# Huguet57/LIMO-Velo

Measured on NVIDIA B200. Metric: matched-points/sec per IESKF iteration (64k-pt sweep, 1M-pt map), higher is better.
Workload: dtype f32 geometry / f64 Jacobian+filter

## Files before the change

limo-velo_b200/csrc/lv_capi.cu:

```cuda
#include <math.h>
#include <stddef.h>
#include <stdio.h>
#include <stdlib.h>
#include <string.h>

#include <string>
#include <vector>

#include "../../include/limovelo_b200.h"
#include "lv_host.h"
#include "lv_internal.h"
#include "lv_predict.h"

using namespace lv;

static_assert(sizeof(lv_iter_log) == sizeof(IterLog), "lv_iter_log must mirror lv::IterLog");
static_assert(LV_MAX_EVALS == kMaxEvals, "log capacity");
static_assert(LV_STATE_LEN == kStateLen && LV_DOF == kDof, "state layout");

static thread_local std::string g_last_error;
static void set_error(const std::string& s) { g_last_error = s; }

#define LV_CUDA(call)                                                                            \
    do {                                                                                         \
// ... 122 lines not shown
}

static void fill_iprm(lv_context* h) {
    h->iprm.R = h->prm.LiDAR_noise;
    h->iprm.D = h->prm.degeneracy_threshold;
    for (int i = 0; i < kN; ++i) h->iprm.limits[i] = h->prm.LIMITS[i];
    h->iprm.max_iter = h->prm.MAX_NUM_ITERS;
    h->iprm.estimate_extrinsics = h->prm.estimate_extrinsics;
}

static MeasureArgs make_measure_args(lv_context* h, const float* d_xyz, int64_t n) {
    MeasureArgs a;
    memset(&a, 0, sizeof(a));
    a.xyz = d_xyz;
    a.n = (int32_t)n;
    a.n_tiles = (int32_t)((n + kMeasureThreads - 1) / kMeasureThreads);
    a.map = map_view(h->map);
    a.ctrl = h->d_ctrl;
    const double md = h->prm.MAX_DIST_PLANE;
    a.gate_d2 = md * md;
    float f = (float)a.gate_d2;
    if ((double)f < a.gate_d2) f = nextafterf(f, INFINITY);
    a.max_d2 = f;
    a.planes_threshold = h->prm.PLANES_THRESHOLD;
    a.estimate_extrinsics = h->prm.estimate_extrinsics;
    a.partials = h->d_partials;
    a.group_rows = h->d_group_rows;
    a.group_tickets = h->d_group_tickets;
    a.nn_a = h->d_nn_a;
    a.nn_b = h->d_nn_b;
    a.hard_list = h->d_hard_list;
    a.hard_seg = hard_segment(h->prm.max_points);
    a.hard_count = h->d_hard_list + (size_t)kHardBuckets * a.hard_seg;
    if (h->prm.sort_queries) {
        a.bin_key = h->d_bin_key; a.bin_val = h->d_bin_val; a.bin_key_in = h->d_bin_key_in; a.bin_val_in = h->d_bin_val_in;
        a.redo_flag = h->d_redo_flag;
        a.sort_tmp = h->d_bin_tmp; a.sort_tmp_bytes = h->bin_tmp_bytes;
        a.sort_bits = 0;
        for (uint32_t sl = h->map.slots; sl > 1; sl >>= 1) a.sort_bits++;
    }
    return a;
}

template <class T>
static cudaError_t ensure(T** p, size_t count) {
    if (*p) return cudaSuccess;
    return cudaMalloc(p, sizeof(T) * count);
}

extern "C" {

const char* lv_last_error(void) { return g_last_error.c_str(); }
const char* lv_version(void) { return "limovelo_b200 0.1 (sm_100a)"; }
int64_t lv_result_bytes(void) { return (int64_t)sizeof(UpdateCtrl); }

#define LV_CREATE_CUDA(call)                                                                     \
    do {                                                                                         \
        cudaError_t e__ = (call);                                                                \
        if (e__ != cudaSuccess) {                                                                \
            char buf__[512];                                                                     \
            snprintf(buf__, sizeof(buf__), "%s:%d: %s -> %s", __FILE__, __LINE__, #call,         \
                     cudaGetErrorString(e__));                                                   \
            lv_destroy(h);                                                                       \
            set_error(buf__);                                                                    \
            return LV_ERR_CUDA;                                                                  \
        }                                                                                        \
    } while (0)

lv_status lv_create(const lv_params* p, lv_handle* out) {
    if (!p || !out) return LV_ERR_ARG;
    *out = nullptr;
    if (p->NUM_MATCH_POINTS != 5) { set_error("NUM_MATCH_POINTS must be 5 (5x3 plane fit)"); return LV_ERR_ARG; }
    if (p->MAX_NUM_ITERS < 0 || p->MAX_NUM_ITERS + 1 > LV_MAX_EVALS) {
        set_error("MAX_NUM_ITERS out of range");
        return LV_ERR_ARG;
    }
    if (!(p->voxel_size > 0.f) || !(p->map_downsample_size > 0.f) || p->max_map_points <= 0 || p->max_points <= 0) {
        set_error("bad capacity / voxel_size / map_downsample_size");
        return LV_ERR_ARG;
    }
    if (p->max_map_points > (1ll << 24) || p->max_points > (1ll << 24)) { set_error("capacity beyond 2^24 points"); return LV_ERR_ARG; }
    if (!(p->MAX_DIST_PLANE > 0.0) || p->MAX_DIST_PLANE > 48.0 * (double)p->map_downsample_size) {
        set_error("MAX_DIST_PLANE must be positive and at most 48 map_downsample_size (ring search bound)");
        return LV_ERR_ARG;
    }
    int ndev = 0;
    if (cudaGetDeviceCount(&ndev) != cudaSuccess || ndev <= 0) {
        set_error("no CUDA device available (there is no CPU fallback)");
        return LV_ERR_CUDA;
    }
    LV_CUDA(cudaSetDevice(p->device));
    lv_context* h = new lv_context();
    h->prm = *p;
    memset(&h->prof, 0, sizeof(h->prof));
    memset(h->logs, 0, sizeof(h->logs));
    memset(&h->map, 0, sizeof(h->map));
    fill_iprm(h);
    if (p->stream) { h->stream = (cudaStream_t)p->stream; h->own_stream = false; }
    else { LV_CREATE_CUDA(cudaStreamCreateWithFlags(&h->stream, cudaStreamNonBlocking)); h->own_stream = true; }
    LV_CREATE_CUDA(map_alloc(h->map, p->max_map_points, p->max_points, p->voxel_size, p->map_downsample_size));
    { int l = 0; LV_CREATE_CUDA(map_clear(h->map, h->stream, &l)); }
    LV_CREATE_CUDA(cudaMalloc(&h->d_sweep, sizeof(float) * 3 * p->max_points));
    LV_CREATE_CUDA(cudaMalloc(&h->d_nn_a, sizeof(int4) * p->max_points));
    LV_CREATE_CUDA(cudaMalloc(&h->d_nn_b, sizeof(int2) * p->max_points));
    LV_CREATE_CUDA(cudaMalloc(&h->d_hard_list, sizeof(uint32_t) * ((size_t)kHardBuckets * hard_segment(p->max_points) + kCounters)));
    LV_CREATE_CUDA(cudaMalloc(&h->d_ref, sizeof(float4) * p->max_points));
    LV_CREATE_CUDA(cudaMalloc(&h->d_redo, sizeof(uint32_t) * (p->max_points + 64)));
// ... 323 lines not shown
        lv_context::UpdateGraph u;
        lv_status s = build_update_graph(h, cap, &u);
        if (s != LV_OK) return s;
        h->graphs.push_back(u);
        g = &h->graphs.back();
    }
    UpdateCtrl* c = h->d_ctrl;
    MeasureJob* job = h->d_job;
    int n32 = (int)n;
    uint32_t* counters = h->d_hard_list + (size_t)kHardBuckets * hard_segment(h->prm.max_points);
    void* args[5] = {&c, &job, &d_xyz, &n32, &counters};
    cudaKernelNodeParams kp = {};
    kp.func = const_cast<void*>(ieskf_begin_kernel_ptr());
    kp.gridDim = dim3(1, 1, 1);
    kp.blockDim = dim3(256, 1, 1);
    kp.kernelParams = args;
    LV_CUDA(cudaGraphExecKernelNodeSetParams(g->exec, g->begin_node, &kp));
    LV_CUDA(cudaGraphLaunch(g->exec, h->stream));
    h->prof.total_launches += 1 + 4 * (h->prm.MAX_NUM_ITERS + 1) + (h->use_reuse ? h->prm.MAX_NUM_ITERS : 0) + (h->prm.sort_queries ? 5 : 0);
    return LV_OK;
}

static lv_status enqueue_update_kernels(lv_context* h, const float* d_xyz, int64_t n, bool as_job) {
    const int pdl = (h->use_pdl && !h->profile) ? 1 : 0;
    uint32_t* counters = h->d_hard_list + (size_t)kHardBuckets * hard_segment(h->prm.max_points);
    LV_CUDA(launch_ieskf_begin(h->d_ctrl, as_job ? h->d_job : nullptr, d_xyz, (int)n, counters, h->stream));
    if (!as_job) h->prof.total_launches += 1;
    MeasureArgs a = update_measure_args(h, d_xyz, n, as_job);
    const int grid = measure_grid((int)n);
    if (a.bin_key) {
        int l = 0;
        LV_CUDA(launch_bin(a, h->stream, pdl, &l));
        if (!as_job) h->prof.total_launches += l;
    }
    for (int e = 0; e <= h->prm.MAX_NUM_ITERS; ++e) {
        EventPair ep;
        bool pr;
        LV_CUDA(launch_measure_timed(h, a, grid, as_job ? 0 : 1, e , (int)(h->update_seq % kNevalsRing), e, pdl));
        pr = prof_begin(h, 1, &ep);
        ep.upd = (int)(h->update_seq % kNevalsRing); ep.slot = e;
        LV_CUDA(launch_ieskf_step(h->d_ctrl, h->iprm, h->d_group_rows, partial_groups(grid), h->stream, pdl));
        if (pr) prof_end(h, &ep);
        if (!as_job) h->prof.total_launches += 4 + ((e > 0 && h->use_reuse) ? 1 : 0);
    }
    if (h->profile) {
        LV_CUDA(cudaMemcpyAsync(&h->h_nevals[h->update_seq % kNevalsRing], &h->d_ctrl->n_evals, sizeof(int32_t),
                                cudaMemcpyDeviceToHost, h->stream));
        h->update_seq++;
    }
    return LV_OK;
}

static lv_status fetch_results(lv_context* h) {
    LV_CUDA(cudaMemcpyAsync(h->h_ctrl, h->d_ctrl, sizeof(UpdateCtrl), cudaMemcpyDeviceToHost, h->stream));
    LV_CUDA(map_fetch_counters(h->map, h->stream));
    LV_CUDA(cudaStreamSynchronize(h->stream));
    const UpdateCtrl* c = h->h_ctrl;
    memcpy(h->x, c->x, sizeof(h->x));
    if (c->status == LV_OK) memcpy(h->P, c->P, sizeof(h->P));
    h->n_evals = c->n_evals;
    memcpy(h->logs, c->logs, sizeof(h->logs));
    h->last_status = c->status;
    h->state_dirty = false;
    h->pending_fetch = false;
    if (c->status == LV_OK && map_status_from_mirror(h) != LV_OK) return LV_ERR_CAPACITY;
    return (lv_status)c->status;
}

lv_status lv_correct(lv_handle h, const float* xyz, int64_t n, double time, lv_iter_log* logs, int32_t* n_evals,
                     double* x_out, double* P_out) {
    if (!h || !xyz || n <= 0) return LV_ERR_ARG;
    if (n_evals) *n_evals = 0;
    if (h->map.empty) return LV_EMPTY_MAP;
    if (n > h->prm.max_points) { set_error("sweep capacity exceeded"); return LV_ERR_CAPACITY; }
    LV_CUDA(cudaSetDevice(h->prm.device));
    LV_CUDA(cudaMemcpyAsync(h->d_sweep, xyz, sizeof(float) * 3 * n, cudaMemcpyHostToDevice, h->stream));
    lv_status s = enqueue_update(h, h->d_sweep, n);
    if (s != LV_OK) return s;
    h->last_sweep = h->d_sweep; h->last_sweep_n = n;
    s = fetch_results(h);
    h->last_time_updated = time;
    if (logs) memcpy(logs, h->logs, sizeof(lv_iter_log) * (size_t)h->n_evals);
    if (n_evals) *n_evals = h->n_evals;
    if (x_out) memcpy(x_out, h->x, sizeof(h->x));
    if (P_out) memcpy(P_out, h->P, sizeof(h->P));
    return s;
}

lv_status lv_correct_device(lv_handle h, const float* d_xyz, int64_t n, double time) {
    if (!h || !d_xyz || n <= 0) return LV_ERR_ARG;
    if (h->map.empty) return LV_EMPTY_MAP;
    LV_CUDA(cudaSetDevice(h->prm.device));
    lv_status s = enqueue_update(h, d_xyz, n);
    h->last_sweep = d_xyz; h->last_sweep_n = n;
    h->last_time_updated = time;
    h->pending_fetch = true;
    return s;
}

lv_status lv_last_logs(lv_handle h, lv_iter_log* logs, int32_t* n_evals) {
    if (!h) return LV_ERR_ARG;
    LV_CUDA(cudaSetDevice(h->prm.device));
    lv_status s = fetch_results(h);
    if (logs) memcpy(logs, h->logs, sizeof(lv_iter_log) * (size_t)h->n_evals);
    if (n_evals) *n_evals = h->n_evals;
    return s;
}
// ... 278 lines not shown
```

limo-velo_b200/csrc/lv_hd.h:

```cpp
#ifndef LV_HD_H_
#define LV_HD_H_

#include <math.h>
#include <stdint.h>

#if defined(__CUDACC__)
#define LV_HD __host__ __device__ __forceinline__
#define LV_HD_NOINLINE __host__ __device__ inline
#else
#define LV_HD inline
#define LV_HD_NOINLINE inline
#endif

namespace lv {

LV_HD float fmul(float a, float b) {
#if defined(__CUDA_ARCH__)
    return __fmul_rn(a, b);
#else
    return a * b;
#endif
}
LV_HD float fadd(float a, float b) {
#if defined(__CUDA_ARCH__)
    return __fadd_rn(a, b);
#else
    return a + b;
#endif
}
LV_HD float fsub(float a, float b) {
#if defined(__CUDA_ARCH__)
    return __fsub_rn(a, b);
#else
    return a - b;
#endif
}
LV_HD float fdiv(float a, float b) {
#if defined(__CUDA_ARCH__)
    return __fdiv_rn(a, b);
#else
    return a / b;
#endif
}
LV_HD float fsqrt(float a) {
#if defined(__CUDA_ARCH__)
    return __fsqrt_rn(a);
#else
    return sqrtf(a);
#endif
}
LV_HD double dmul(double a, double b) {
#if defined(__CUDA_ARCH__)
    return __dmul_rn(a, b);
#else
    return a * b;
#endif
}
LV_HD double dadd(double a, double b) {
#if defined(__CUDA_ARCH__)
    return __dadd_rn(a, b);
#else
    return a + b;
#endif
}
// ... 18 lines not shown
```

limo-velo_b200/csrc/lv_ieskf.h:

```cpp
#ifndef LV_IESKF_H_
#define LV_IESKF_H_

#include "lv_point_math.h"

namespace lv {

#ifndef LV_TK
#define LV_TK(k)
#endif
#ifndef LV_CK
#define LV_CK(k)
#endif

enum { kN = 23, kAug = 46, kMaxEvals = 8 };

struct IeskfParams {
    double R;
    double D;
    double limits[kN];
    int32_t max_iter;
    int32_t estimate_extrinsics;
};

struct IterLog {
    int64_t n_matches;
    int32_t converged;
    int32_t degenerate;
    double HTH[144];
    double HTh[12];
    double dx[kN];
    double x_after[kStateLen];
};

struct UpdateCtrl {
    int32_t iter;
    int32_t t;
    int32_t done;
    int32_t status;
    int32_t n_evals;
    int32_t pad_[3];
    double x_prop[kStateLen];
    double P_prop[kN * kN];
    double x[kStateLen];
    double P[kN * kN];
    Frame frame;
    IterLog logs[kMaxEvals];
    double P_j[kN * kN];
    double dx_new[kN];
};

struct PrepWork {
    double x[kStateLen], xp[kStateLen];
    double P[kN * kN];
    double dx[kN], dx_new[kN];
    double J[3][9];
};

struct IeskfWork {
    double x[kStateLen], xp[kStateLen];
    double P[kN * kN];
    double M1[12 * 25];
    double Kx[kN * 12];
    double Kh[kN];
    double HTH[144], HTh[12];
    double dx[kN], dx_new[kN], dxs[kN], dnd[kN];
    double J[3][9];
    double L[kN * kN];
    double xn[kStateLen];
    double pivval;
    int64_t n_matches;
    int32_t piv;
    int32_t finish;
    int32_t abort_;
    int32_t degen;
    int32_t eval_idx;
    int32_t n_evals, t, iter;
};

struct ExecSerial {
    int tid, nthreads;
    LV_HD ExecSerial() : tid(0), nthreads(1) {}
    LV_HD void sync() {}
    LV_HD bool is_task(int) const { return true; }
    LV_HD void solve_12x25(double* M, int32_t* s_piv, double* s_pivval);
    LV_HD void pivot(const double* M, int w, int k, int n, int32_t* s_piv, double* s_pivval) {
        int p = k;
        double best = fabs(M[k * w + k]);
        for (int i = k + 1; i < n; ++i) {
            const double v = fabs(M[i * w + k]);
            if (v > best) { best = v; p = i; }
        }
        *s_piv = p;
        *s_pivval = M[p * w + k];
    }
};
#if defined(__CUDACC__)
struct ExecBlock {
    int tid, nthreads;
    __device__ __forceinline__ ExecBlock() : tid(threadIdx.x), nthreads(blockDim.x) {}
    __device__ __forceinline__ void sync() { __syncthreads(); }
    __device__ __forceinline__ bool is_task(int k) const { return tid == 32 * k; }
    __device__ __forceinline__ void pivot(const double* M, int w, int k, int n, int32_t* s_piv, double* s_pivval) {
        if (tid < 32) {
            const int row = k + tid;
            double v = row < n ? fabs(M[row * w + k]) : -1.0;
            int r = row < n ? row : 0x7fffffff;
#pragma unroll
            for (int s = 16; s > 0; s >>= 1) {
                const double ov = __shfl_xor_sync(0xffffffffu, v, s);
                const int orow = __shfl_xor_sync(0xffffffffu, r, s);
                if (ov > v || (ov == v && orow < r)) { v = ov; r = orow; }
            }
            if (tid == 0) { *s_piv = r; *s_pivval = M[r * w + k]; }
        }
    }
#if defined(LV_GJ_SMEM)
    __device__ __noinline__ void solve_12x25(double* M, int32_t*, double*) {
        if (tid < 32) {
            const int lane = tid;
            const bool act = lane < 25;
            if (lane == 0) LV_TK(48);
#pragma unroll 1
            for (int k = 0; k < 12; ++k) {
                int p = k;
                double best = fabs(M[k * 25 + k]);
#pragma unroll 1
                for (int i = k + 1; i < 12; ++i) {
                    const double v = fabs(M[i * 25 + k]);
                    if (v > best) { best = v; p = i; }
                }
                const double ipv = 1.0 / M[p * 25 + k];
                __syncwarp();
                double ck = 0.0;
                if (act) {
                    const double a = M[k * 25 + lane], b = M[p * 25 + lane];
                    if (p != k) M[p * 25 + lane] = a;
                    ck = b * ipv;
                    M[k * 25 + lane] = ck;
                }
                __syncwarp();
                double m[12];
#pragma unroll
                for (int i = 0; i < 12; ++i) m[i] = M[i * 25 + k];
                __syncwarp();
                if (act) {
#pragma unroll
                    for (int i = 0; i < 12; ++i)
                        if (i != k) M[i * 25 + lane] -= m[i] * ck;
                }
                __syncwarp();
            }
            if (lane == 0) { LV_TK(49); LV_TK(52); }
        }
        __syncthreads();
    }
#else
    __device__ __noinline__ void solve_12x25(double* M, int32_t*, double*) {
        if (tid < 32) {
            const int lane = tid;
            const unsigned full = 0xffffffffu;
            double col[12];
#pragma unroll
            for (int i = 0; i < 12; ++i) col[i] = lane < 25 ? M[i * 25 + lane] : 0.0;
            if (lane == 0) LV_TK(48);
#pragma unroll
            for (int k = 0; k < 12; ++k) {
                double v[12];
                int r[12];
#pragma unroll
                for (int i = k; i < 12; ++i) { v[i] = fabs(col[i]); r[i] = i; }
#pragma unroll
                for (int s = 1; s < 12; s *= 2)
#pragma unroll
                    for (int i = k; i + s < 12; i += 2 * s)
                        if (v[i + s] > v[i]) { v[i] = v[i + s]; r[i] = r[i + s]; }
                const int p = __shfl_sync(full, r[k], k);
                double ck = col[k];
#pragma unroll
                for (int i = k + 1; i < 12; ++i)
                    if (i == p) { const double tmp = col[i]; col[i] = ck; ck = tmp; }
                const double ipv = 1.0 / __shfl_sync(full, ck, k);
                ck *= ipv;
                col[k] = ck;
#pragma unroll
                for (int i = 0; i < 12; ++i)
                    if (i != k) col[i] -= __shfl_sync(full, col[i], k) * ck;
            }
            if (lane == 0) LV_TK(49);
#pragma unroll
            for (int i = 0; i < 12; ++i)
                if (lane >= 12 && lane < 25) M[i * 25 + lane] = col[i];
            if (lane == 0) LV_TK(52);
        }
        __syncthreads();
    }
#endif
};
#endif

#define LV_PAR(i, n) for (int i = ex.tid; i < (n); i += ex.nthreads)

template <class Ex>
LV_HD_NOINLINE void gj_solve(Ex& ex, double* M, int n, int w, int32_t* s_piv, double* s_pivval) {
    for (int k = 0; k < n; ++k) {
        ex.pivot(M, w, k, n, s_piv, s_pivval);
        ex.sync();
        const int p = *s_piv;
        const double ipv = 1.0 / *s_pivval;
        LV_PAR(jj, w - k) {
            const int j = k + jj;
            const double a = M[k * w + j], b = M[p * w + j];
            if (p != k) M[p * w + j] = a;
            M[k * w + j] = b * ipv;
        }
        ex.sync();
        const int ncols = w - k - 1;
        LV_PAR(it, (n - 1) * ncols) {
            int i = it / ncols;
            const int j = k + 1 + (it - i * ncols);
            if (i >= k) ++i;
            M[i * w + j] -= M[i * w + k] * M[k * w + j];
        }
        ex.sync();
    }
}

LV_HD void ExecSerial::solve_12x25(double* M, int32_t* s_piv, double* s_pivval) {
    gj_solve(*this, M, 12, 25, s_piv, s_pivval);
}

LV_HD int jblock_idx(int b) { return b < 2 ? 3 + 3 * b : 21; }
LV_HD int jblock_dim(int b) { return b < 2 ? 3 : 2; }

template <class Ex>
LV_HD void apply_rows3(Ex& ex, double* dst, const double* src, const double (*J)[9], int cols, int stride) {
    LV_PAR(it, 3 * cols) {
        const int b = it / cols, i = it - b * cols;
        const int idx = jblock_idx(b), d = jblock_dim(b);
        double v[3], r[3];
        for (int c = 0; c < d; ++c) v[c] = src[(idx + c) * stride + i];
        for (int a = 0; a < d; ++a) {
            double s = 0;
            for (int c = 0; c < d; ++c) s += J[b][a * d + c] * v[c];
            r[a] = s;
        }
        for (int a = 0; a < d; ++a) dst[(idx + a) * stride + i] = r[a];
    }
}
template <class Ex>
LV_HD void apply_cols3(Ex& ex, double* M, const double (*J)[9], int rows, int stride) {
    LV_PAR(it, 3 * rows) {
        const int b = it / rows, i = it - b * rows;
        const int idx = jblock_idx(b), d = jblock_dim(b);
        double v[3], r[3];
        for (int c = 0; c < d; ++c) v[c] = M[i * stride + idx + c];
        for (int a = 0; a < d; ++a) {
            double s = 0;
            for (int c = 0; c < d; ++c) s += v[c] * J[b][a * d + c];
            r[a] = s;
        }
        for (int a = 0; a < d; ++a) M[i * stride + idx + a] = r[a];
    }
}

LV_HD_NOINLINE void sym_eig6(const double* Ain, double* ev, double* V) {
    const int n = 6;
    double A[36];
    for (int i = 0; i < 36; ++i) { A[i] = Ain[i]; V[i] = (i % 7 == 0) ? 1.0 : 0.0; }
    for (int sweep = 0; sweep < 60; ++sweep) {
        double off = 0, diag = 0;
        for (int i = 0; i < n; ++i) {
            diag += A[i * n + i] * A[i * n + i];
            for (int j = i + 1; j < n; ++j) off += A[i * n + j] * A[i * n + j];
        }
        if (off <= 1e-30 * diag || off == 0.0) break;
        for (int p = 0; p < n; ++p)
            for (int q = p + 1; q < n; ++q) {
                const double apq = A[p * n + q];
                if (apq == 0.0) continue;
                const double theta = (A[q * n + q] - A[p * n + p]) / (2 * apq);
                const double t = (theta >= 0 ? 1.0 : -1.0) / (fabs(theta) + sqrt(theta * theta + 1));
                const double c = 1 / sqrt(t * t + 1), s = t * c;
                for (int k = 0; k < n; ++k) {
                    const double akp = A[k * n + p], akq = A[k * n + q];
                    A[k * n + p] = c * akp - s * akq;
                    A[k * n + q] = s * akp + c * akq;
                }
                for (int k = 0; k < n; ++k) {
                    const double apk = A[p * n + k], aqk = A[q * n + k];
                    A[p * n + k] = c * apk - s * aqk;
                    A[q * n + k] = s * apk + c * aqk;
                }
                for (int k = 0; k < n; ++k) {
                    const double vkp = V[k * n + p], vkq = V[k * n + q];
                    V[k * n + p] = c * vkp - s * vkq;
                    V[k * n + q] = s * vkp + c * vkq;
                }
            }
    }
    double Vs[36];
    bool used[6] = {false, false, false, false, false, false};
    for (int j = 0; j < n; ++j) {
        int src = -1;
        for (int c = 0; c < n; ++c)
            if (!used[c] && (src < 0 || A[c * n + c] < A[src * n + src])) src = c;
        used[src] = true;
        ev[j] = A[src * n + src];
        int imax = 0;
        for (int k = 1; k < n; ++k)
            if (fabs(V[k * n + src]) > fabs(V[imax * n + src])) imax = k;
        const double sg = V[imax * n + src] < 0 ? -1.0 : 1.0;
        for (int k = 0; k < n; ++k) Vs[k * n + j] = sg * V[k * n + src];
    }
    for (int i = 0; i < 36; ++i) V[i] = Vs[i];
}

LV_HD_NOINLINE void degenerate_mask(const double* HTH, double D, const double* dxs, double* dnd) {
    double A6[36], ev[6], V[36], sel[36];
    for (int i = 0; i < 6; ++i)
        for (int j = 0; j < 6; ++j) A6[i * 6 + j] = HTH[i * 12 + j];
    sym_eig6(A6, ev, V);
    double prod = 1;
    for (int i = 0; i < 6; ++i) prod *= ev[i];
    if (prod < 1e-20)
        for (int i = 0; i < 36; ++i) V[i] = (i % 7 == 0) ? 1.0 : 0.0;
    for (int i = 0; i < 36; ++i) sel[i] = V[i];
    for (int j = 0; j < 6; ++j)
        if (ev[j] < D)
            for (int c = 0; c < 6; ++c) sel[j * 6 + c] = 0;
    double t[6];
    for (int i = 0; i < 6; ++i) {
        double s = 0;
        for (int j = 0; j < 6; ++j) s += sel[i * 6 + j] * dxs[j];
        t[i] = s;
    }
    double M[6 * 7];
    for (int i = 0; i < 6; ++i) {
        for (int j = 0; j < 6; ++j) M[i * 7 + j] = V[i * 6 + j];
        M[i * 7 + 6] = t[i];
    }
    for (int k = 0; k < 6; ++k) {
        int p = k;
        for (int i = k + 1; i < 6; ++i)
            if (fabs(M[i * 7 + k]) > fabs(M[p * 7 + k])) p = i;
        if (p != k)
            for (int j = 0; j < 7; ++j) { const double tmp = M[k * 7 + j]; M[k * 7 + j] = M[p * 7 + j]; M[p * 7 + j] = tmp; }
        const double pv = M[k * 7 + k];
        for (int j = k; j < 7; ++j) M[k * 7 + j] /= pv;
        for (int i = 0; i < 6; ++i) {
            if (i == k) continue;
            const double f = M[i * 7 + k];
            for (int j = k; j < 7; ++j) M[i * 7 + j] -= f * M[k * 7 + j];
        }
    }
    for (int i = 0; i < 6; ++i) dnd[i] = M[i * 7 + 6];
}

LV_HD bool all_eigs_above(const double* HTH, double D) {
    double Lc[36];
    for (int i = 0; i < 6; ++i)
        for (int j = 0; j <= i; ++j) {
            double s = HTH[i * 12 + j] - (i == j ? D : 0.0);
            for (int k = 0; k < j; ++k) s -= Lc[i * 6 + k] * Lc[j * 6 + k];
            if (i == j) {
                if (!(s > 0.0)) return false;
                Lc[i * 6 + i] = sqrt(s);
            } else {
                Lc[i * 6 + j] = s / Lc[j * 6 + j];
            }
        }
    return true;
}

LV_HD_NOINLINE void jblock(int b, const double* d, const double* x_now, const double* x_prop, double* J) {
    if (b < 2) {
        const Mat3d Jt = mat3_transpose(A_matrix(load_vec3(d + 3 + 3 * b)));
        for (int i = 0; i < 9; ++i) J[i] = Jt.m[i];
    } else {
        s2_J(load_vec3(x_now + kGrav), load_vec3(x_prop + kGrav), d[21], d[22], J);
    }
}

template <class Ex>
LV_HD_NOINLINE void ieskf_prepare(Ex& ex, UpdateCtrl* c, PrepWork* w) {
    const int n = kN;
    LV_PAR(i, n * n) w->P[i] = c->P_prop[i];
    LV_PAR(i, kStateLen) { w->x[i] = c->x[i]; w->xp[i] = c->x_prop[i]; }
    ex.sync();
    for (int b = 0; b < 3; ++b)
        if (ex.is_task(b)) {
            const int idx = jblock_idx(b), d = jblock_dim(b);
            if (b < 2) {
                const int q = b == 0 ? kRot : kOffR;
                store_vec3(w->dx + idx, so3_log(quat_mul(quat_conj(load_quat(w->xp + q)), load_quat(w->x + q))));
            } else {
                s2_boxminus(load_vec3(w->x + kGrav), load_vec3(w->xp + kGrav), w->dx + 21);
            }
            jblock(b, w->dx, w->x, w->xp, w->J[b]);
            for (int a = 0; a < d; ++a) {
                double s = 0;
                for (int k = 0; k < d; ++k) s += w->J[b][a * d + k] * w->dx[idx + k];
                w->dx_new[idx + a] = s;
            }
        }
    if (ex.is_task(3)) {
        const int lin[5][2] = {{0, kPos}, {9, kOffT}, {12, kVel}, {15, kBg}, {18, kBa}};
        for (int g = 0; g < 5; ++g)
            for (int i = 0; i < 3; ++i) {
                const double v = w->x[lin[g][1] + i] - w->xp[lin[g][1] + i];
                w->dx[lin[g][0] + i] = v;
                w->dx_new[lin[g][0] + i] = v;
            }
    }
    ex.sync();
    apply_rows3(ex, w->P, w->P, w->J, n, n);
    ex.sync();
    apply_cols3(ex, w->P, w->J, n, n);
    ex.sync();
    LV_PAR(i, n * n) c->P_j[i] = w->P[i];
    LV_PAR(i, n) c->dx_new[i] = w->dx_new[i];
}

template <class Ex>
LV_HD void ieskf_load(Ex& ex, const UpdateCtrl* c, IeskfWork* w) {
    LV_PAR(i, kN * kN) w->P[i] = c->P_j[i];
    LV_PAR(i, kN) w->dx_new[i] = c->dx_new[i];
    LV_PAR(i, kStateLen) { w->x[i] = c->x[i]; w->xp[i] = c->x_prop[i]; }
    if (ex.tid == 0) {
        w->n_evals = c->n_evals;
        w->eval_idx = w->n_evals < kMaxEvals ? w->n_evals : kMaxEvals - 1;
        w->t = c->t;
        w->iter = c->iter;
    }
}

template <class Ex>
LV_HD_NOINLINE void ieskf_step(Ex& ex, const IeskfParams& prm, UpdateCtrl* c, IeskfWork* w) {
    const int n = kN;
    IterLog* lg = &c->logs[w->eval_idx];
    if (w->n_matches < n) {
        if (ex.tid == 0) {
            lg->n_matches = w->n_matches;
            c->status = 2;
            c->done = 1;
        }
        return;
    }
    LV_CK(3);

    const double invR = 1.0 / prm.R;
    LV_PAR(it, 12 * 25) {
        const int i = it / 25, j = it - i * 25;
        double v;
        if (j < 12) {
            double s = 0;
            for (int k = 0; k < 12; ++k) s += w->HTH[i * 12 + k] * w->P[k * n + j];
            v = s * invR + (i == j ? 1.0 : 0.0);
        } else if (j < 24) {
            v = w->HTH[i * 12 + (j - 12)];
        } else {
            v = w->HTh[i];
        }
        w->M1[it] = v;
    }
    ex.sync();
    LV_CK(5);
    if (ex.is_task(1)) { LV_TK(50); w->degen = all_eigs_above(w->HTH, prm.D) ? 0 : 1; LV_TK(51); }
    ex.solve_12x25(w->M1, &w->piv, &w->pivval);
    LV_CK(6);
    LV_PAR(it, n * 13) {
        const int i = it / 13, j = it - i * 13;
        double s = 0;
        for (int k = 0; k < 12; ++k) s += w->P[i * n + k] * w->M1[k * 25 + 12 + j];
        s *= invR;
        if (j < 12) w->Kx[i * 12 + j] = s; else w->Kh[i] = s;
    }
    ex.sync();
    LV_PAR(i, n) {
        double s = 0;
        for (int j = 0; j < 12; ++j) s += w->Kx[i * 12 + j] * w->dx_new[j];
        w->dxs[i] = w->Kh[i] + s - w->dx_new[i];
        w->dnd[i] = w->dxs[i];
    }
    ex.sync();
    LV_CK(7);

    LV_PAR(i, 144) lg->HTH[i] = w->HTH[i];
    LV_PAR(i, 12) lg->HTh[i] = w->HTh[i];
    LV_PAR(i, n) lg->dx[i] = w->dxs[i];
    LV_TK(24 + (ex.tid >> 5));
    if (ex.is_task(0)) {
        for (int i = 0; i < 3; ++i) w->xn[kPos + i] = w->x[kPos + i] + w->dnd[i];
        for (int i = 0; i < 3; ++i) w->xn[kOffT + i] = w->x[kOffT + i] + w->dnd[9 + i];
        const Quatd q = quat_mul(load_quat(w->x + kRot), so3_exp(load_vec3(w->dnd + 3), 0.5));
        const Quatd ql = quat_mul(load_quat(w->x + kOffR), so3_exp(load_vec3(w->dnd + 6), 0.5));
        store_quat(w->xn + kRot, q);
        store_quat(w->xn + kOffR, ql);
        const Mat3d R = quat_to_rot(q), Ri = quat_to_rot(quat_conj(q));
        const Mat3d RL = quat_to_rot(ql), RLi = quat_to_rot(quat_conj(ql));
        Rt32 X, IL;
        for (int i = 0; i < 9; ++i) { X.R[i] = (float)R.m[i]; IL.R[i] = (float)RL.m[i]; }
        for (int i = 0; i < 3; ++i) { X.t[i] = (float)w->xn[kPos + i]; IL.t[i] = (float)w->xn[kOffT + i]; }
        for (int i = 0; i < 9; ++i) { c->frame.R_inv[i] = Ri.m[i]; c->frame.RLI_inv[i] = RLi.m[i]; }
        c->frame.lidar_to_world = rt_mul(X, IL);
        c->frame.world_to_lidar = rt_mul(rt_inv(IL), rt_inv(X));
        c->frame.lidar_to_imu = IL;
    }
    if (ex.is_task(2)) store_vec3(w->xn + kGrav, s2_boxplus(load_vec3(w->x + kGrav), w->dnd[21], w->dnd[22]));
    if (ex.is_task(3)) {
        for (int i = 0; i < 9; ++i) w->xn[kVel + i] = w->x[kVel + i] + w->dnd[12 + i];
        int conv = 1;
        for (int i = 0; i < n; ++i)
            if (fabs(w->dxs[i]) > prm.limits[i]) { conv = 0; break; }
        const int t = w->t + conv;
        if (!t && w->iter == prm.max_iter - 2) conv = 1;
        lg->n_matches = w->n_matches;
        lg->converged = conv;
        c->t = t;
        c->n_evals = w->n_evals + 1;
        w->finish = (t > 1 || w->iter == prm.max_iter - 1) ? 1 : 0;
        c->iter = w->iter + 1;
    }
    if ((ex.tid & 31) == 0 && ex.tid < 160) LV_TK(32 + (ex.tid >> 5));
    ex.sync();
    if (w->degen) {
        if (ex.tid == 0) {
            degenerate_mask(w->HTH, prm.D, w->dxs, w->dnd);
            for (int i = 0; i < kStateLen; ++i) w->xn[i] = w->x[i];
            state_boxplus(w->xn, w->dnd);
            make_frame(w->xn, &c->frame);
        }
        ex.sync();
    }
    if (ex.is_task(1)) lg->degenerate = w->degen;
    LV_PAR(i, kStateLen) {
        const double v = w->xn[i];
        w->x[i] = v;
        c->x[i] = v;
        lg->x_after[i] = v;
    }
    ex.sync();
    LV_CK(8);
    if (!w->finish) return;

    LV_PAR(i, n * n) w->L[i] = w->P[i];
    for (int b = 0; b < 3; ++b)
        if (ex.is_task(b)) jblock(b, w->dxs, w->x, w->xp, w->J[b]);
    ex.sync();
    apply_rows3(ex, w->L, w->P, w->J, n, n);
    apply_rows3(ex, w->Kx, w->Kx, w->J, 12, 12);
    ex.sync();
    apply_cols3(ex, w->L, w->J, n, n);
    apply_cols3(ex, w->P, w->J, n, n);
    ex.sync();
    LV_PAR(it, n * n) {
        const int i = it / n, j = it - i * n;
        double s = 0;
        for (int k = 0; k < 12; ++k) s += w->Kx[i * 12 + k] * w->P[k * n + j];
        c->P[it] = w->L[it] - s;
    }
    if (ex.tid == 0) c->done = 1;
    ex.sync();
    LV_CK(9);
}

template <class Ex>
LV_HD void ieskf_begin(Ex& ex, UpdateCtrl* c) {
    LV_PAR(i, kStateLen) c->x_prop[i] = c->x[i];
    LV_PAR(i, kN * kN) c->P_prop[i] = c->P[i];
    if (ex.tid == 0) {
        c->iter = -1;
        c->t = 0;
        c->done = 0;
        c->status = 0;
        c->n_evals = 0;
        make_frame(c->x, &c->frame);
    }
    ex.sync();
}

}
#endif
```

limo-velo_b200/csrc/lv_internal.h:

```cpp
#ifndef LV_INTERNAL_H_
#define LV_INTERNAL_H_

#include <cuda_runtime.h>
#include <stdint.h>

#include "../../include/limovelo_b200.h"
#include "lv_ieskf.h"
#include "lv_voxel_search.h"

namespace lv {

enum { kMeasureThreads = 128, kPartialStride = 96, kStepThreads = 512, kPartialGroup = 32 };
inline int partial_groups(int grid) { return (grid + kPartialGroup - 1) / kPartialGroup; }
enum { kHardBuckets = 32, kCounters = 4 + kHardBuckets };
inline uint32_t hard_segment(int64_t n) { return (uint32_t)((n + kHardBuckets - 1) / kHardBuckets + 160); }

struct MeasureJob {
    const float* xyz;
    int32_t n;
    int32_t n_tiles;
};

struct MeasureArgs {
    const float* xyz;
    int32_t n;
    int32_t n_tiles;
    const MeasureJob* job;
    VoxelMapView map;
    const UpdateCtrl* ctrl;
    UpdateCtrl* prep;
    float max_d2;
    double gate_d2;
    float planes_threshold;
    int32_t estimate_extrinsics;
    double* partials;
    double* group_rows;
    uint32_t* group_tickets;
    uint8_t* valid;
    int32_t* nn_idx;
    float* nn_sqd;
    float* plane;
    float* dist;
    float* g_world;
    double* rows;
    int4* nn_a;
    int2* nn_b;
    uint32_t* hard_list;
    uint32_t hard_seg;
    uint32_t* hard_count;
    float4* ref;
    uint32_t* redo_list;
    const uint32_t* bin_key;
    const uint32_t* bin_val;
    uint32_t* bin_key_in;
    uint32_t* bin_val_in;
    uint8_t* redo_flag;
    void* sort_tmp;
    size_t sort_tmp_bytes;
    int32_t sort_bits;
};

struct MapBuffers {
    MapGrid grid;
    uint4* table;
    uint32_t slots;
// ... 72 lines not shown
```

limo-velo_b200/csrc/lv_measure.cu:

```cuda
#include <stdio.h>
#include <stdlib.h>
#include <string.h>

#ifdef LV_STEP_TIMING
__device__ unsigned long long g_probes[2];
#ifdef __CUDA_ARCH__
#define LV_PROBE_COUNT() do { atomicAdd(&g_probes[0], 1ull); } while (0)
#endif
#endif
#ifdef LV_STEP_TIMING
__device__ long long g_step_clk[64];
#ifdef __CUDA_ARCH__
#define LV_CK(k) do { if (threadIdx.x == 0) g_step_clk[k] = clock64(); } while (0)
#define LV_TK(k) do { g_step_clk[k] = clock64(); } while (0)
#define LV_FK(k) do { if (threadIdx.x == 0 && blockIdx.x == 1) g_step_clk[k] = clock64(); } while (0)
#endif
#endif
#ifndef LV_FK
#define LV_FK(k)
#endif

#include <cub/device/device_radix_sort.cuh>

#include "lv_internal.h"
// ... 598 lines not shown
        if (tid < 91) {
            double v[kPartialGroup];
#pragma unroll
            for (int r = 0; r < kPartialGroup; ++r) v[r] = r0 + r < r1 ? __ldcg(a.partials + (size_t)(r0 + r) * kPartialStride + tid) : 0.0;
            double sum = 0.0;
#pragma unroll
            for (int r = 0; r < kPartialGroup; ++r) sum += v[r];
            a.group_rows[(size_t)grp * kPartialStride + tid] = sum;
        }
    }
    LV_FK(63);
    LV_TL_END(4);
}

__device__ void reduce_partials_block(const double* partials, int n_partials, double* s_tmp ,
                                      double* HTH, double* HTh, int64_t* nm) {
    const int warp = threadIdx.x >> 5, lane = threadIdx.x & 31, nwarps = blockDim.x >> 5;
    double a0 = 0, a1 = 0, a2 = 0;
    for (int b = warp; b < n_partials; b += 8 * nwarps) {
        double v[8][3];
#pragma unroll
        for (int r = 0; r < 8; ++r) {
            const int row = b + r * nwarps;
            const double* p = partials + (size_t)row * kPartialStride;
            const bool in = row < n_partials;
            v[r][0] = in ? p[lane] : 0.0;
            v[r][1] = in ? p[lane + 32] : 0.0;
            v[r][2] = in ? p[lane + 64] : 0.0;
        }
#pragma unroll
        for (int r = 0; r < 8; ++r) { a0 += v[r][0]; a1 += v[r][1]; a2 += v[r][2]; }
    }
    s_tmp[warp * 96 + lane] = a0;
    s_tmp[warp * 96 + lane + 32] = a1;
    s_tmp[warp * 96 + lane + 64] = a2;
    __syncthreads();
    if (threadIdx.x < 91) {
        double s = 0;
        for (int w = 0; w < nwarps; ++w) s += s_tmp[w * 96 + threadIdx.x];
        const int e = threadIdx.x;
        if (e < 78) {
            const int i = c_pair_a[e], j = c_pair_b[e];
            HTH[i * 12 + j] = s;
            HTH[j * 12 + i] = s;
        } else if (e < 90) {
            HTh[e - 78] = s;
        } else {
            *nm = (int64_t)(s + 0.5);
        }
    }
    __syncthreads();
}

__global__ void __launch_bounds__(kStepThreads) lv_ieskf_step_kernel(UpdateCtrl* c, const IeskfParams prm,
                                                                     const double* partials, int n_partials) {
    static_assert(kStepThreads >= 99 && 2 * kStepThreads >= kN * kN, "one pass for the state, two for P_j");
    LV_TL_SCHED();
    const int t = threadIdx.x;
    const int done = c->done;
    double sv = 0.0;
    if (t < 26) sv = c->x[t];
    else if (t < 52) sv = c->x_prop[t - 26];
    int cv = 0;
    if (t >= 96 && t < 99) cv = t == 96 ? c->n_evals : (t == 97 ? c->t : c->iter);
    pdl_wait();
    pdl_trigger();
    LV_TL_WORK(c, 5);
    if (done) return;
    __shared__ IeskfWork w;
    __shared__ double s_tmp[(kStepThreads / 32) * 96];
    ExecBlock ex;
    LV_CK(0);
    const double pj0 = t < kN * kN ? c->P_j[t] : 0.0;
    const double pj1 = t + kStepThreads < kN * kN ? c->P_j[t + kStepThreads] : 0.0;
    if (t >= 52 && t < 75) sv = c->dx_new[t - 52];
    LV_CK(1);
    reduce_partials_block(partials, n_partials, s_tmp, w.HTH, w.HTh, &w.n_matches);
    if (t < kN * kN) w.P[t] = pj0;
    if (t + kStepThreads < kN * kN) w.P[t + kStepThreads] = pj1;
    if (t < 26) w.x[t] = sv;
    else if (t < 52) w.xp[t - 26] = sv;
    else if (t < 75) w.dx_new[t - 52] = sv;
    if (t == 96) { w.n_evals = cv; w.eval_idx = cv < kMaxEvals ? cv : kMaxEvals - 1; }
    if (t == 97) w.t = cv;
    if (t == 98) w.iter = cv;
    __syncthreads();
    LV_CK(2);
    ieskf_step(ex, prm, c, &w);
    LV_TL_END(5);
}

__global__ void __launch_bounds__(kStepThreads) lv_reduce_partials_kernel(const double* partials, int n_partials,
                                                                          double* out) {
    __shared__ double s_tmp[(kStepThreads / 32) * 96];
    __shared__ double HTH[144], HTh[12];
    __shared__ int64_t nm;
    reduce_partials_block(partials, n_partials, s_tmp, HTH, HTh, &nm);
    for (int i = threadIdx.x; i < 144; i += blockDim.x) out[i] = HTH[i];
    if (threadIdx.x < 12) out[144 + threadIdx.x] = HTh[threadIdx.x];
    if (threadIdx.x == 0) out[156] = (double)nm;
}

__global__ void __launch_bounds__(256) lv_ieskf_begin_kernel(UpdateCtrl* c, MeasureJob* job, const float* xyz, int n,
                                                             uint32_t* counters) {
    pdl_trigger();
    if (counters && threadIdx.x < kCounters) counters[threadIdx.x] = 0u;
    if (job && threadIdx.x == 0) {
        job->xyz = xyz;
        job->n = n;
        job->n_tiles = (n + kMeasureThreads - 1) / kMeasureThreads;
    }
    ExecBlock ex;
    ieskf_begin(ex, c);
}

__global__ void __launch_bounds__(256) lv_predict_kernel(UpdateCtrl* c, const PredictNoise noise, const double* __restrict__ imu, int k) {
    __shared__ PredictWork w;
    ExecBlock ex;
    LV_PAR(i, kStateLen) w.x[i] = c->x[i];
    LV_PAR(i, kN * kN) w.P[i] = c->P[i];
    ex.sync();
    for (int s = 0; s < k; ++s) predict_step(ex, noise, imu + 7 * s, imu + 7 * s + 3, imu[7 * s + 6], &w);
    LV_PAR(i, kStateLen) c->x[i] = w.x[i];
    LV_PAR(i, kN * kN) c->P[i] = w.P[i];
}

__global__ void lv_set_frame_kernel(UpdateCtrl* c) {
    if (threadIdx.x == 0) {
        make_frame(c->x, &c->frame);
        c->done = 0;
    }
}

__global__ void lv_l2_flush_kernel(uint4* buf, size_t n16) {
    const size_t stride = (size_t)gridDim.x * blockDim.x;
// ... 146 lines not shown
```

Measured before the change: 1.242 billion.

## Precompute P11 inverse in prepare and use pivot-free SPD solve in IESKF step

Moves the inverse of the leading 12x12 block of P, and the product of the lower P rows with that inverse, into the once-per-update prepare stage. Each step then forms R*P11^-1 + HTH directly and solves it with a symmetric positive definite Gauss-Jordan elimination that skips pivoting, which drops the HTH*P matmul and the pivot search. The step kernel block also shrinks to 256 threads, the pose frame work is split across two warps, and cold paths are marked noinline. The host fetch is cut to exclude the prep data. Dropping pivoting assumes the matrices stay well conditioned, and the change in algebra can move numerical results.

Measured after the change: 1.426 billion, median of 6. +14.8%, better.

```diff
diff --git a/limo-velo_b200/csrc/lv_capi.cu b/limo-velo_b200/csrc/lv_capi.cu
--- a/limo-velo_b200/csrc/lv_capi.cu
+++ b/limo-velo_b200/csrc/lv_capi.cu
@@ -198,7 +198,8 @@
 
 const char* lv_last_error(void) { return g_last_error.c_str(); }
 const char* lv_version(void) { return "limovelo_b200 0.1 (sm_100a)"; }
-int64_t lv_result_bytes(void) { return (int64_t)sizeof(UpdateCtrl); }
+static const size_t kResultBytes = offsetof(UpdateCtrl, prep);
+int64_t lv_result_bytes(void) { return (int64_t)kResultBytes; }
 
 #define LV_CREATE_CUDA(call)                                                                     \
     do {                                                                                         \
@@ -628,7 +629,7 @@
 }
 
 static lv_status fetch_results(lv_context* h) {
-    LV_CUDA(cudaMemcpyAsync(h->h_ctrl, h->d_ctrl, sizeof(UpdateCtrl), cudaMemcpyDeviceToHost, h->stream));
+    LV_CUDA(cudaMemcpyAsync(h->h_ctrl, h->d_ctrl, kResultBytes, cudaMemcpyDeviceToHost, h->stream));
     LV_CUDA(map_fetch_counters(h->map, h->stream));
     LV_CUDA(cudaStreamSynchronize(h->stream));
     const UpdateCtrl* c = h->h_ctrl;
diff --git a/limo-velo_b200/csrc/lv_hd.h b/limo-velo_b200/csrc/lv_hd.h
--- a/limo-velo_b200/csrc/lv_hd.h
+++ b/limo-velo_b200/csrc/lv_hd.h
@@ -7,9 +7,11 @@
 #if defined(__CUDACC__)
 #define LV_HD __host__ __device__ __forceinline__
 #define LV_HD_NOINLINE __host__ __device__ inline
+#define LV_HD_COLD __host__ __device__ inline __noinline__
 #else
 #define LV_HD inline
 #define LV_HD_NOINLINE inline
+#define LV_HD_COLD inline
 #endif
 
 namespace lv {
diff --git a/limo-velo_b200/csrc/lv_ieskf.h b/limo-velo_b200/csrc/lv_ieskf.h
--- a/limo-velo_b200/csrc/lv_ieskf.h
+++ b/limo-velo_b200/csrc/lv_ieskf.h
@@ -30,6 +30,13 @@
     double HTh[12];
     double dx[kN];
     double x_after[kStateLen];
+};
+
+struct StepPrep {
+    double P_j[kN * kN];
+    double dx_new[kN];
+    double P11inv[144];
+    double T[11 * 12];
 };
 
 struct UpdateCtrl {
@@ -45,8 +52,7 @@
     double P[kN * kN];
     Frame frame;
     IterLog logs[kMaxEvals];
-    double P_j[kN * kN];
-    double dx_new[kN];
+    StepPrep prep;
 };
 
 struct PrepWork {
@@ -54,24 +60,23 @@
     double P[kN * kN];
     double dx[kN], dx_new[kN];
     double J[3][9];
+    double M[12 * 24];
 };
 
 struct IeskfWork {
     double x[kStateLen], xp[kStateLen];
-    double P[kN * kN];
-    double M1[12 * 25];
+    StepPrep p;
+    double M[12 * 25];
     double Kx[kN * 12];
     double Kh[kN];
     double HTH[144], HTh[12];
-    double dx[kN], dx_new[kN], dxs[kN], dnd[kN];
+    double dxs[kN], dnd[kN];
     double J[3][9];
     double L[kN * kN];
     double xn[kStateLen];
-    double pivval;
+    Rt32 X, IL;
     int64_t n_matches;
-    int32_t piv;
     int32_t finish;
-    int32_t abort_;
     int32_t degen;
     int32_t eval_idx;
     int32_t n_evals, t, iter;
@@ -82,16 +87,18 @@
     LV_HD ExecSerial() : tid(0), nthreads(1) {}
     LV_HD void sync() {}
     LV_HD bool is_task(int) const { return true; }
-    LV_HD void solve_12x25(double* M, int32_t* s_piv, double* s_pivval);
-    LV_HD void pivot(const double* M, int w, int k, int n, int32_t* s_piv, double* s_pivval) {
-        int p = k;
-        double best = fabs(M[k * w + k]);
-        for (int i = k + 1; i < n; ++i) {
-            const double v = fabs(M[i * w + k]);
-            if (v > best) { best = v; p = i; }
-        }
-        *s_piv = p;
-        *s_pivval = M[p * w + k];
+    LV_HD void solve_spd12(double* M, int w) {
+        for (int k = 0; k < 12; ++k) {
+            double m[12];
+            for (int i = 0; i < 12; ++i) m[i] = M[i * w + k];
+            const double ipv = 1.0 / m[k];
+            for (int j = 0; j < w; ++j) {
+                const double ck = M[k * w + j] * ipv;
+                M[k * w + j] = ck;
+                for (int i = 0; i < 12; ++i)
+                    if (i != k) M[i * w + j] -= m[i] * ck;
+            }
+        }
     }
 };
 #if defined(__CUDACC__)
@@ -100,87 +107,18 @@
     __device__ __forceinline__ ExecBlock() : tid(threadIdx.x), nthreads(blockDim.x) {}
     __device__ __forceinline__ void sync() { __syncthreads(); }
     __device__ __forceinline__ bool is_task(int k) const { return tid == 32 * k; }
-    __device__ __forceinline__ void pivot(const double* M, int w, int k, int n, int32_t* s_piv, double* s_pivval) {
-        if (tid < 32) {
-            const int row = k + tid;
-            double v = row < n ? fabs(M[row * w + k]) : -1.0;
-            int r = row < n ? row : 0x7fffffff;
-#pragma unroll
-            for (int s = 16; s > 0; s >>= 1) {
-                const double ov = __shfl_xor_sync(0xffffffffu, v, s);
-                const int orow = __shfl_xor_sync(0xffffffffu, r, s);
-                if (ov > v || (ov == v && orow < r)) { v = ov; r = orow; }
-            }
-            if (tid == 0) { *s_piv = r; *s_pivval = M[r * w + k]; }
-        }
-    }
-#if defined(LV_GJ_SMEM)
-    __device__ __noinline__ void solve_12x25(double* M, int32_t*, double*) {
-        if (tid < 32) {
-            const int lane = tid;
-            const bool act = lane < 25;
-            if (lane == 0) LV_TK(48);
-#pragma unroll 1
-            for (int k = 0; k < 12; ++k) {
-                int p = k;
-                double best = fabs(M[k * 25 + k]);
-#pragma unroll 1
-                for (int i = k + 1; i < 12; ++i) {
-                    const double v = fabs(M[i * 25 + k]);
-                    if (v > best) { best = v; p = i; }
-                }
-                const double ipv = 1.0 / M[p * 25 + k];
-                __syncwarp();
-                double ck = 0.0;
-                if (act) {
-                    const double a = M[k * 25 + lane], b = M[p * 25 + lane];
-                    if (p != k) M[p * 25 + lane] = a;
-                    ck = b * ipv;
-                    M[k * 25 + lane] = ck;
-                }
-                __syncwarp();
-                double m[12];
-#pragma unroll
-                for (int i = 0; i < 12; ++i) m[i] = M[i * 25 + k];
-                __syncwarp();
-                if (act) {
-#pragma unroll
-                    for (int i = 0; i < 12; ++i)
-                        if (i != k) M[i * 25 + lane] -= m[i] * ck;
-                }
-                __syncwarp();
-            }
-            if (lane == 0) { LV_TK(49); LV_TK(52); }
-        }
-        __syncthreads();
-    }
-#else
-    __device__ __noinline__ void solve_12x25(double* M, int32_t*, double*) {
+    __device__ __forceinline__ void solve_spd12(double* M, int w) {
         if (tid < 32) {
             const int lane = tid;
             const unsigned full = 0xffffffffu;
             double col[12];
 #pragma unroll
-            for (int i = 0; i < 12; ++i) col[i] = lane < 25 ? M[i * 25 + lane] : 0.0;
+            for (int i = 0; i < 12; ++i) col[i] = lane < w ? M[i * w + lane] : 0.0;
             if (lane == 0) LV_TK(48);
 #pragma unroll
             for (int k = 0; k < 12; ++k) {
-                double v[12];
-                int r[12];
-#pragma unroll
-                for (int i = k; i < 12; ++i) { v[i] = fabs(col[i]); r[i] = i; }
-#pragma unroll
-                for (int s = 1; s < 12; s *= 2)
-#pragma unroll
-                    for (int i = k; i + s < 12; i += 2 * s)
-                        if (v[i + s] > v[i]) { v[i] = v[i + s]; r[i] = r[i + s]; }
-                const int p = __shfl_sync(full, r[k], k);
-                double ck = col[k];
-#pragma unroll
-                for (int i = k + 1; i < 12; ++i)
-                    if (i == p) { const double tmp = col[i]; col[i] = ck; ck = tmp; }
-                const double ipv = 1.0 / __shfl_sync(full, ck, k);
-                ck *= ipv;
+                const double ipv = 1.0 / __shfl_sync(full, col[k], k);
+                const double ck = col[k] * ipv;
                 col[k] = ck;
 #pragma unroll
                 for (int i = 0; i < 12; ++i)
@@ -189,45 +127,15 @@
             if (lane == 0) LV_TK(49);
 #pragma unroll
             for (int i = 0; i < 12; ++i)
-                if (lane >= 12 && lane < 25) M[i * 25 + lane] = col[i];
+                if (lane >= 12 && lane < w) M[i * w + lane] = col[i];
             if (lane == 0) LV_TK(52);
         }
         __syncthreads();
     }
+};
 #endif
-};
-#endif
 
 #define LV_PAR(i, n) for (int i = ex.tid; i < (n); i += ex.nthreads)
-
-template <class Ex>
-LV_HD_NOINLINE void gj_solve(Ex& ex, double* M, int n, int w, int32_t* s_piv, double* s_pivval) {
-    for (int k = 0; k < n; ++k) {
-        ex.pivot(M, w, k, n, s_piv, s_pivval);
-        ex.sync();
-        const int p = *s_piv;
-        const double ipv = 1.0 / *s_pivval;
-        LV_PAR(jj, w - k) {
-            const int j = k + jj;
-            const double a = M[k * w + j], b = M[p * w + j];
-            if (p != k) M[p * w + j] = a;
-            M[k * w + j] = b * ipv;
-        }
-        ex.sync();
-        const int ncols = w - k - 1;
-        LV_PAR(it, (n - 1) * ncols) {
-            int i = it / ncols;
-            const int j = k + 1 + (it - i * ncols);
-            if (i >= k) ++i;
-            M[i * w + j] -= M[i * w + k] * M[k * w + j];
-        }
-        ex.sync();
-    }
-}
-
-LV_HD void ExecSerial::solve_12x25(double* M, int32_t* s_piv, double* s_pivval) {
-    gj_solve(*this, M, 12, 25, s_piv, s_pivval);
-}
 
 LV_HD int jblock_idx(int b) { return b < 2 ? 3 + 3 * b : 21; }
 LV_HD int jblock_dim(int b) { return b < 2 ? 3 : 2; }
@@ -263,7 +171,7 @@
     }
 }
 
-LV_HD_NOINLINE void sym_eig6(const double* Ain, double* ev, double* V) {
+LV_HD_COLD void sym_eig6(const double* Ain, double* ev, double* V) {
     const int n = 6;
     double A[36];
     for (int i = 0; i < 36; ++i) { A[i] = Ain[i]; V[i] = (i % 7 == 0) ? 1.0 : 0.0; }
@@ -315,7 +223,7 @@
     for (int i = 0; i < 36; ++i) V[i] = Vs[i];
 }
 
-LV_HD_NOINLINE void degenerate_mask(const double* HTH, double D, const double* dxs, double* dnd) {
+LV_HD_COLD void degenerate_mask(const double* HTH, double D, const double* dxs, double* dnd) {
     double A6[36], ev[6], V[36], sel[36];
     for (int i = 0; i < 6; ++i)
         for (int j = 0; j < 6; ++j) A6[i * 6 + j] = HTH[i * 12 + j];
@@ -372,7 +280,7 @@
     return true;
 }
 
-LV_HD_NOINLINE void jblock(int b, const double* d, const double* x_now, const double* x_prop, double* J) {
+LV_HD_COLD void jblock(int b, const double* d, const double* x_now, const double* x_prop, double* J) {
     if (b < 2) {
         const Mat3d Jt = mat3_transpose(A_matrix(load_vec3(d + 3 + 3 * b)));
         for (int i = 0; i < 9; ++i) J[i] = Jt.m[i];
@@ -381,9 +289,17 @@
     }
 }
 
+LV_HD_COLD void degenerate_redo(double D, IeskfWork* w, Frame* frame) {
+    degenerate_mask(w->HTH, D, w->dxs, w->dnd);
+    for (int i = 0; i < kStateLen; ++i) w->xn[i] = w->x[i];
+    state_boxplus(w->xn, w->dnd);
+    make_frame(w->xn, frame);
+}
+
 template <class Ex>
 LV_HD_NOINLINE void ieskf_prepare(Ex& ex, UpdateCtrl* c, PrepWork* w) {
     const int n = kN;
+    StepPrep* out = &c->prep;
     LV_PAR(i, n * n) w->P[i] = c->P_prop[i];
     LV_PAR(i, kStateLen) { w->x[i] = c->x[i]; w->xp[i] = c->x_prop[i]; }
     ex.sync();
@@ -417,14 +333,26 @@
     ex.sync();
     apply_cols3(ex, w->P, w->J, n, n);
     ex.sync();
-    LV_PAR(i, n * n) c->P_j[i] = w->P[i];
-    LV_PAR(i, n) c->dx_new[i] = w->dx_new[i];
+    LV_PAR(it, 12 * 24) {
+        const int i = it / 24, j = it - i * 24;
+        w->M[it] = j < 12 ? w->P[i * n + j] : (j - 12 == i ? 1.0 : 0.0);
+    }
+    LV_PAR(i, n * n) out->P_j[i] = w->P[i];
+    LV_PAR(i, n) out->dx_new[i] = w->dx_new[i];
+    ex.sync();
+    ex.solve_spd12(w->M, 24);
+    LV_PAR(i, 144) out->P11inv[i] = w->M[(i / 12) * 24 + 12 + i % 12];
+    LV_PAR(it, 11 * 12) {
+        const int i = it / 12, j = it - i * 12;
+        double s = 0;
+        for (int k = 0; k < 12; ++k) s += w->P[(12 + i) * n + k] * w->M[k * 24 + 12 + j];
+        out->T[it] = s;
+    }
 }
 
 template <class Ex>
 LV_HD void ieskf_load(Ex& ex, const UpdateCtrl* c, IeskfWork* w) {
-    LV_PAR(i, kN * kN) w->P[i] = c->P_j[i];
-    LV_PAR(i, kN) w->dx_new[i] = c->dx_new[i];
+    LV_PAR(i, (int)(sizeof(StepPrep) / sizeof(double))) reinterpret_cast<double*>(&w->p)[i] = reinterpret_cast<const double*>(&c->prep)[i];
     LV_PAR(i, kStateLen) { w->x[i] = c->x[i]; w->xp[i] = c->x_prop[i]; }
     if (ex.tid == 0) {
         w->n_evals = c->n_evals;
@@ -437,6 +365,7 @@
 template <class Ex>
 LV_HD_NOINLINE void ieskf_step(Ex& ex, const IeskfParams& prm, UpdateCtrl* c, IeskfWork* w) {
     const int n = kN;
+    const double* dx_new = w->p.dx_new;
     IterLog* lg = &c->logs[w->eval_idx];
     if (w->n_matches < n) {
         if (ex.tid == 0) {
@@ -448,38 +377,35 @@
     }
     LV_CK(3);
 
-    const double invR = 1.0 / prm.R;
     LV_PAR(it, 12 * 25) {
         const int i = it / 25, j = it - i * 25;
         double v;
-        if (j < 12) {
-            double s = 0;
-            for (int k = 0; k < 12; ++k) s += w->HTH[i * 12 + k] * w->P[k * n + j];
-            v = s * invR + (i == j ? 1.0 : 0.0);
-        } else if (j < 24) {
-            v = w->HTH[i * 12 + (j - 12)];
-        } else {
-            v = w->HTh[i];
-        }
-        w->M1[it] = v;
+        if (j < 12) v = prm.R * w->p.P11inv[i * 12 + j] + w->HTH[i * 12 + j];
+        else if (j < 24) v = w->HTH[i * 12 + (j - 12)];
+        else v = w->HTh[i];
+        w->M[it] = v;
     }
     ex.sync();
     LV_CK(5);
     if (ex.is_task(1)) { LV_TK(50); w->degen = all_eigs_above(w->HTH, prm.D) ? 0 : 1; LV_TK(51); }
-    ex.solve_12x25(w->M1, &w->piv, &w->pivval);
+    ex.solve_spd12(w->M, 25);
     LV_CK(6);
     LV_PAR(it, n * 13) {
         const int i = it / 13, j = it - i * 13;
-        double s = 0;
-        for (int k = 0; k < 12; ++k) s += w->P[i * n + k] * w->M1[k * 25 + 12 + j];
-        s *= invR;
+        double s;
+        if (i < 12) {
+            s = w->M[i * 25 + 12 + j];
+        } else {
+            s = 0;
+            for (int k = 0; k < 12; ++k) s += w->p.T[(i - 12) * 12 + k] * w->M[k * 25 + 12 + j];
+        }
         if (j < 12) w->Kx[i * 12 + j] = s; else w->Kh[i] = s;
     }
     ex.sync();
     LV_PAR(i, n) {
         double s = 0;
-        for (int j = 0; j < 12; ++j) s += w->Kx[i * 12 + j] * w->dx_new[j];
-        w->dxs[i] = w->Kh[i] + s - w->dx_new[i];
+        for (int j = 0; j < 12; ++j) s += w->Kx[i * 12 + j] * dx_new[j];
+        w->dxs[i] = w->Kh[i] + s - dx_new[i];
         w->dnd[i] = w->dxs[i];
     }
     ex.sync();
@@ -489,23 +415,20 @@
     LV_PAR(i, 12) lg->HTh[i] = w->HTh[i];
     LV_PAR(i, n) lg->dx[i] = w->dxs[i];
     LV_TK(24 + (ex.tid >> 5));
-    if (ex.is_task(0)) {
-        for (int i = 0; i < 3; ++i) w->xn[kPos + i] = w->x[kPos + i] + w->dnd[i];
-        for (int i = 0; i < 3; ++i) w->xn[kOffT + i] = w->x[kOffT + i] + w->dnd[9 + i];
-        const Quatd q = quat_mul(load_quat(w->x + kRot), so3_exp(load_vec3(w->dnd + 3), 0.5));
-        const Quatd ql = quat_mul(load_quat(w->x + kOffR), so3_exp(load_vec3(w->dnd + 6), 0.5));
-        store_quat(w->xn + kRot, q);
-        store_quat(w->xn + kOffR, ql);
-        const Mat3d R = quat_to_rot(q), Ri = quat_to_rot(quat_conj(q));
-        const Mat3d RL = quat_to_rot(ql), RLi = quat_to_rot(quat_conj(ql));
-        Rt32 X, IL;
-        for (int i = 0; i < 9; ++i) { X.R[i] = (float)R.m[i]; IL.R[i] = (float)RL.m[i]; }
-        for (int i = 0; i < 3; ++i) { X.t[i] = (float)w->xn[kPos + i]; IL.t[i] = (float)w->xn[kOffT + i]; }
-        for (int i = 0; i < 9; ++i) { c->frame.R_inv[i] = Ri.m[i]; c->frame.RLI_inv[i] = RLi.m[i]; }
-        c->frame.lidar_to_world = rt_mul(X, IL);
-        c->frame.world_to_lidar = rt_mul(rt_inv(IL), rt_inv(X));
-        c->frame.lidar_to_imu = IL;
-    }
+#pragma unroll 1
+    for (int b = 0; b < 2; ++b)
+        if (ex.is_task(b)) {
+            const int qo = b == 0 ? kRot : kOffR, to = b == 0 ? kPos : kOffT;
+            for (int i = 0; i < 3; ++i) w->xn[to + i] = w->x[to + i] + w->dnd[9 * b + i];
+            const Quatd q = quat_mul(load_quat(w->x + qo), so3_exp(load_vec3(w->dnd + 3 + 3 * b), 0.5));
+            store_quat(w->xn + qo, q);
+            const Mat3d R = quat_to_rot(q), Ri = quat_to_rot(quat_conj(q));
+            Rt32& X = b == 0 ? w->X : w->IL;
+            for (int i = 0; i < 9; ++i) X.R[i] = (float)R.m[i];
+            for (int i = 0; i < 3; ++i) X.t[i] = (float)w->xn[to + i];
+            double* dst = b == 0 ? c->frame.R_inv : c->frame.RLI_inv;
+            for (int i = 0; i < 9; ++i) dst[i] = Ri.m[i];
+        }
     if (ex.is_task(2)) store_vec3(w->xn + kGrav, s2_boxplus(load_vec3(w->x + kGrav), w->dnd[21], w->dnd[22]));
     if (ex.is_task(3)) {
         for (int i = 0; i < 9; ++i) w->xn[kVel + i] = w->x[kVel + i] + w->dnd[12 + i];
@@ -523,13 +446,13 @@
     }
     if ((ex.tid & 31) == 0 && ex.tid < 160) LV_TK(32 + (ex.tid >> 5));
     ex.sync();
+    if (ex.is_task(0)) {
+        c->frame.lidar_to_world = rt_mul(w->X, w->IL);
+        c->frame.world_to_lidar = rt_mul(rt_inv(w->IL), rt_inv(w->X));
+        c->frame.lidar_to_imu = w->IL;
+    }
     if (w->degen) {
-        if (ex.tid == 0) {
-            degenerate_mask(w->HTH, prm.D, w->dxs, w->dnd);
-            for (int i = 0; i < kStateLen; ++i) w->xn[i] = w->x[i];
-            state_boxplus(w->xn, w->dnd);
-            make_frame(w->xn, &c->frame);
-        }
+        if (ex.tid == 0) degenerate_redo(prm.D, w, &c->frame);
         ex.sync();
     }
     if (ex.is_task(1)) lg->degenerate = w->degen;
@@ -543,20 +466,21 @@
     LV_CK(8);
     if (!w->finish) return;
 
-    LV_PAR(i, n * n) w->L[i] = w->P[i];
+    double* Pj = w->p.P_j;
+    LV_PAR(i, n * n) w->L[i] = Pj[i];
     for (int b = 0; b < 3; ++b)
         if (ex.is_task(b)) jblock(b, w->dxs, w->x, w->xp, w->J[b]);
     ex.sync();
-    apply_rows3(ex, w->L, w->P, w->J, n, n);
+    apply_rows3(ex, w->L, Pj, w->J, n, n);
     apply_rows3(ex, w->Kx, w->Kx, w->J, 12, 12);
     ex.sync();
     apply_cols3(ex, w->L, w->J, n, n);
-    apply_cols3(ex, w->P, w->J, n, n);
+    apply_cols3(ex, Pj, w->J, n, n);
     ex.sync();
     LV_PAR(it, n * n) {
         const int i = it / n, j = it - i * n;
         double s = 0;
-        for (int k = 0; k < 12; ++k) s += w->Kx[i * 12 + k] * w->P[k * n + j];
+        for (int k = 0; k < 12; ++k) s += w->Kx[i * 12 + k] * Pj[k * n + j];
         c->P[it] = w->L[it] - s;
     }
     if (ex.tid == 0) c->done = 1;
diff --git a/limo-velo_b200/csrc/lv_internal.h b/limo-velo_b200/csrc/lv_internal.h
--- a/limo-velo_b200/csrc/lv_internal.h
+++ b/limo-velo_b200/csrc/lv_internal.h
@@ -10,7 +10,7 @@
 
 namespace lv {
 
-enum { kMeasureThreads = 128, kPartialStride = 96, kStepThreads = 512, kPartialGroup = 32 };
+enum { kMeasureThreads = 128, kPartialStride = 96, kStepThreads = 256, kPartialGroup = 32 };
 inline int partial_groups(int grid) { return (grid + kPartialGroup - 1) / kPartialGroup; }
 enum { kHardBuckets = 32, kCounters = 4 + kHardBuckets };
 inline uint32_t hard_segment(int64_t n) { return (uint32_t)((n + kHardBuckets - 1) / kHardBuckets + 160); }
diff --git a/limo-velo_b200/csrc/lv_measure.cu b/limo-velo_b200/csrc/lv_measure.cu
--- a/limo-velo_b200/csrc/lv_measure.cu
+++ b/limo-velo_b200/csrc/lv_measure.cu
@@ -674,9 +674,11 @@
     __syncthreads();
 }
 
-__global__ void __launch_bounds__(kStepThreads) lv_ieskf_step_kernel(UpdateCtrl* c, const IeskfParams prm,
+__global__ void __launch_bounds__(kStepThreads, 1) lv_ieskf_step_kernel(UpdateCtrl* c, const IeskfParams prm,
                                                                      const double* partials, int n_partials) {
-    static_assert(kStepThreads >= 99 && 2 * kStepThreads >= kN * kN, "one pass for the state, two for P_j");
+    constexpr int kPrepWords = (int)(sizeof(StepPrep) / sizeof(double));
+    constexpr int kPrepLoads = (kPrepWords + kStepThreads - 1) / kStepThreads;
+    static_assert(kStepThreads >= 99, "one pass for the state and the counters");
     LV_TL_SCHED();
     const int t = threadIdx.x;
     const int done = c->done;
@@ -693,16 +695,18 @@
     __shared__ double s_tmp[(kStepThreads / 32) * 96];
     ExecBlock ex;
     LV_CK(0);
-    const double pj0 = t < kN * kN ? c->P_j[t] : 0.0;
-    const double pj1 = t + kStepThreads < kN * kN ? c->P_j[t + kStepThreads] : 0.0;
-    if (t >= 52 && t < 75) sv = c->dx_new[t - 52];
+    const double* src = reinterpret_cast<const double*>(&c->prep);
+    double pv[kPrepLoads];
+#pragma unroll
+    for (int r = 0; r < kPrepLoads; ++r) pv[r] = t + r * kStepThreads < kPrepWords ? src[t + r * kStepThreads] : 0.0;
     LV_CK(1);
     reduce_partials_block(partials, n_partials, s_tmp, w.HTH, w.HTh, &w.n_matches);
-    if (t < kN * kN) w.P[t] = pj0;
-    if (t + kStepThreads < kN * kN) w.P[t + kStepThreads] = pj1;
+    double* dst = reinterpret_cast<double*>(&w.p);
+#pragma unroll
+    for (int r = 0; r < kPrepLoads; ++r)
+        if (t + r * kStepThreads < kPrepWords) dst[t + r * kStepThreads] = pv[r];
     if (t < 26) w.x[t] = sv;
     else if (t < 52) w.xp[t - 26] = sv;
-    else if (t < 75) w.dx_new[t - 52] = sv;
     if (t == 96) { w.n_evals = cv; w.eval_idx = cv < kMaxEvals ? cv : kMaxEvals - 1; }
     if (t == 97) w.t = cv;
     if (t == 98) w.iter = cv;
```
